# fani-lab/OpeNTF

Hardware: AMD Instinct MI355X
Metric: teams/sec (train) bnn_emb d=128 on DBLP (higher is better)
Workload: dtype f32 (fp16x3 split products, f32 accumulate)

## Files before the change

opentf_amd/csrc/ntf_device.h:

```cpp
#pragma once
#include <hip/hip_runtime.h>
#include <stdint.h>
#include "ntf_kernels.h"

namespace ntf {

typedef float f32x16 __attribute__((ext_vector_type(16)));
typedef float f32x4 __attribute__((ext_vector_type(4)));

__device__ __forceinline__ uint32_t fmix32(uint32_t x) {
    x ^= x >> 16; x *= 0x85ebca6bu; x ^= x >> 13; x *= 0xc2b2ae35u; x ^= x >> 16;
    return x;
}

__device__ __forceinline__ uint32_t sign_word(uint32_t k0, uint32_t k1, uint32_t r, uint32_t cb) {
    uint32_t h = fmix32(r * 0x9E3779B1u + k0);
    return fmix32(h ^ (cb * 0x85EBCA77u + k1));
}
__device__ __forceinline__ float sign_hash(uint32_t k0, uint32_t k1, uint32_t r, uint32_t c) {
    return ((sign_word(k0, k1, r, c >> 5) >> (c & 31)) & 1u) ? -1.0f : 1.0f;
}
__device__ __forceinline__ float sign_at(const SignSpec& s, int64_t r, int64_t c) {
    if (s.inj) return s.inj[r * s.ld + c];
    return sign_hash(s.k0, s.k1, (uint32_t)r, (uint32_t)c);
// ... 115 lines not shown
    const float denom = fmaf(__builtin_amdgcn_sqrtf(v), inv_bc2_sqrt, eps);
    p = p - (lr_over_bc1 * m) * __builtin_amdgcn_rcpf(denom);
#endif
}

__device__ __forceinline__ float wave_reduce_sum(float v) {
#pragma unroll
    for (int o = 32; o > 0; o >>= 1) v += __shfl_xor(v, o, 64);
    return v;
}
__device__ __forceinline__ double wave_reduce_sum_d(double v) {
#pragma unroll
    for (int o = 32; o > 0; o >>= 1) v += __shfl_xor(v, o, 64);
    return v;
}
__device__ __forceinline__ float block_reduce_sum(float v) {
    __shared__ float sh_f[16];
    v = wave_reduce_sum(v);
    const int w = threadIdx.x >> 6, nw = (blockDim.x + 63) >> 6;
    __syncthreads();
    if ((threadIdx.x & 63) == 0) sh_f[w] = v;
    __syncthreads();
    float s = 0.f;
    if (threadIdx.x == 0) for (int i = 0; i < nw; ++i) s += sh_f[i];
    return s;
}
__device__ __forceinline__ double block_reduce_sum_d(double v) {
    __shared__ double sh_d[16];
    v = wave_reduce_sum_d(v);
    const int w = threadIdx.x >> 6, nw = (blockDim.x + 63) >> 6;
// ... 10 lines not shown
```

opentf_amd/csrc/ntf_engine.hip:

```cpp
#include "../../include/opentf_amd.h"
#include "ntf_kernels.h"
#include "ntf_fused.h"
#include "ntf_head.h"
#include "ntf_host.h"
#include "ntf_select.h"

#include <algorithm>
#include <cmath>
#include <cstdio>
#include <cstdlib>
#include <cstring>
#include <string>
#include <vector>

using namespace ntf;

static thread_local std::string g_create_error;

struct LayerInfo {
    int in = 0, out = 0;
    int64_t off[4] = {0, 0, 0, 0};
    int64_t nw() const { return (int64_t)in * out; }
};

// ... 91 lines not shown
    int64_t pre_used = 0;
    int eval_chain = 0; bool chain_valid = false; double* d_chain = nullptr;
    bool join_pending = false;
    bool pre_rotated = false;
    bool fin_pend = false; NormalSpec fin_eps; float fin_klw = 0.f;
    int (*cb_fn)(int32_t, void*) = nullptr; void* cb_user = nullptr;
    bool pend_valid = false; FusedDw pend; NormalSpec pend_eps_b; float pend_klw_b = 0.f; int pend_chunks = 0;
    std::vector<int32_t> ub_entries; void* ub_host[2] = {nullptr, nullptr}; char* ub_dev[2] = {nullptr, nullptr}; hipEvent_t ub_ev[2] = {nullptr, nullptr};
    bool ub_used[2] = {false, false}; size_t ub_cap = 0; int ub_slot = 0; int ub_nsup[2] = {0, 0}; double ub_total[2] = {0, 0};
    uint16_t* pl_mu = nullptr; uint16_t* pl_wp = nullptr;
    hipStream_t st2 = nullptr;
    hipEvent_t ev_chunk = nullptr, ev_side = nullptr;
    hipStream_t st3 = nullptr; hipEvent_t ev_fork = nullptr, ev_join = nullptr;
    hipStream_t st4 = nullptr; hipEvent_t ev_aux = nullptr;
    int side_bwd = 1;
    bool ep = false; int ep_lo = 0, Mg = 0, ep_world = 1;
    bool ep_side = false;
    int ep_open = 0; StepCtx ep_ctx;
};

static int join_side(ntf_engine* e);

struct Scope {
    ntf_engine* e; int fam; hipEvent_t a = nullptr, b = nullptr;
    bool on() const {
        const bool fwd = fam == F_OUT_FUSED_FWD || fam == F_OUT_FWD, dw = fam == F_OUT_FUSED_DW || fam == F_OUT_BWD_DW;
        return e->timing == 1 || (e->timing == 2 && (fwd || dw)) || (e->timing == 3 && fwd) || (e->timing == 4 && dw);
    }
    Scope(ntf_engine* e_, int f) : e(e_), fam(f) {
        if (!on()) return;
// ... 67 lines not shown
    if (const char* hp = getenv("NTF_HEAD_PREFETCH")) e->head_prefetch = atoi(hp);
    if (const char* pf = getenv("NTF_PREFETCH")) e->prefetch = atoi(pf);
    if (const char* hd = getenv("NTF_HEAD")) e->head = atoi(hd);
    if (const char* mb = getenv("NTF_MERGE_BIAS")) e->merge_bias = atoi(mb);
    if (const char* sw = getenv("NTF_L0_SWEEP")) e->l0_sweep = atoi(sw);
    if (const char* fp = getenv("NTF_FNN_PIPE")) e->fnn_pipe = atoi(fp);
    if (const char* mh = getenv("NTF_MH_HEAD")) e->mh_head = atoi(mh);
    if (const char* ek = getenv("NTF_EVAL_KERNEL")) e->eval_kernel = atoi(ek);
    if (const char* nf = getenv("NTF_INFER_F32")) e->infer_f32 = atoi(nf);
    if (const char* mc = getenv("NTF_INFER_MC")) e->infer_mc = atoi(mc);
    if (const char* mb = getenv("NTF_INFER_MC_BYTES")) e->infer_mc_bytes = atoll(mb);
    if (const char* fc = getenv("NTF_F32_COPY_MERGED")) e->f32_copy_merged = atoi(fc);
    if (const char* eh = getenv("NTF_EP_HEAD_PREFETCH")) e->ep_head_prefetch = atoi(eh);
    if (const char* dr = getenv("NTF_DP_RANGES")) e->dp_ranges = atoi(dr);
    if (const char* ds = getenv("NTF_DP_SIDE_BWD")) e->dp_side_bwd = atoi(ds);
    if (const char* sb = getenv("NTF_SIDE_BWD")) e->side_bwd = atoi(sb);
    if (cfg->stream) e->st = (hipStream_t)cfg->stream;
    else { if (hipStreamCreate(&e->st) != hipSuccess) { g_create_error = "hipStreamCreate failed"; delete e; return NTF_EHIP; } e->own_stream = true; }
    int64_t off = 0;
    auto seg = [&](int64_t n) { int64_t o = off; off += (n + 63) / 64 * 64; return o; };
    e->layers.resize(e->L);
    for (int l = 0; l < e->L; ++l) {
        LayerInfo& li = e->layers[l];
        li.in = cfg->dims[l]; li.out = cfg->dims[l + 1];
        li.off[NTF_P_WEIGHT] = seg(li.nw());
        li.off[NTF_P_BIAS] = seg(li.out);
        if (cfg->bayesian) { li.off[NTF_P_RHO_WEIGHT] = seg(li.nw()); li.off[NTF_P_RHO_BIAS] = seg(li.out); }
        if (l < e->L - 1) e->maxhid = std::max(e->maxhid, li.out);
    }
    e->n_params = off;
// ... 17 lines not shown
    const int B = cfg->max_batch, M = cfg->dims[e->L];
    int rc = NTF_OK;
    auto A = [&](int r) { if (rc == NTF_OK) rc = r; };
    A(dev_alloc(e, &e->P, off)); A(dev_alloc(e, &e->G, off)); A(dev_alloc(e, &e->M1, off)); A(dev_alloc(e, &e->V2, off));
    A(dev_alloc(e, &e->d_rows, B)); for (int k = 0; k < 2; ++k) A(dev_alloc(e, &e->d_neg_set[k], (int64_t)B * std::max(1, cfg->ns)));
    e->act.assign(e->L, nullptr);
    for (int l = (cfg->input_mode == NTF_INPUT_MULTIHOT ? 1 : 0); l < e->L; ++l) A(dev_alloc(e, &e->act[l], (int64_t)B * cfg->dims[l]));
    A(dev_alloc(e, &e->Zout, (int64_t)B * M)); A(dev_alloc(e, &e->dZout, (int64_t)((M + 255) / 256 * 256) * fused_ldb(B)));
    if (e->maxhid) { A(dev_alloc(e, &e->Zh, (int64_t)B * e->maxhid)); A(dev_alloc(e, &e->dAct[0], (int64_t)B * e->maxhid)); A(dev_alloc(e, &e->dAct[1], (int64_t)B * e->maxhid)); }
    e->Wp.assign(e->L, nullptr); e->bp.assign(e->L, nullptr);
    if (cfg->bayesian) for (int l = 0; l < e->L; ++l) { A(dev_alloc(e, &e->Wp[l], e->layers[l].nw())); A(dev_alloc(e, &e->bp[l], e->layers[l].out)); }
    A(dev_alloc(e, &e->partial, (int64_t)B * std::max(loss_dense_nchunk(M), fused_loss_slots(M)))); A(dev_alloc(e, &e->row_fix, B));
    if (cfg->bayesian && cfg->input_mode == NTF_INPUT_MULTIHOT) A(dev_alloc(e, &e->l0_touched, (int64_t)(cfg->dims[0] + 255) / 256 * 256));
    A(dev_alloc(e, &e->d_loss, 4)); A(dev_alloc(e, &e->d_kl, 4)); A(dev_alloc(e, &e->d_chain, 2)); A(dev_alloc(e, &e->d_acc, 2)); A(dev_alloc(e, &e->d_acc_steps, 2));
    A(dev_alloc(e, &e->ent_mc, B)); A(dev_alloc(e, &e->ent_mean, B)); A(dev_alloc(e, &e->gemm_slab, kGemmSlabFloats));
    if (rc == NTF_OK && fused_ok(e)) {
        A(dev_alloc(e, &e->dh_slab, fused_dh_slab_floats(B, e->layers[e->L - 1].in, M)));
        for (int k = 0; k < 2; ++k) A(dev_alloc(e, &e->fws_set[k], (int64_t)fused_workspace_bytes(B, e->layers[e->L - 1].in, M)));
        e->fws = e->fws_set[0];
        if (cfg->mfma != NTF_MFMA_F32 && e->layers[e->L - 1].in == 128) {
            A(dev_alloc(e, &e->pl_mu, fused_planes_elems(M, 128)));
            if (cfg->bayesian) A(dev_alloc(e, &e->pl_wp, fused_planes_elems(M, 128)));
            if (rc == NTF_OK) { hipMemsetAsync(e->pl_mu, 0, (size_t)fused_planes_elems(M, 128) * 2, e->st); if (e->pl_wp) hipMemsetAsync(e->pl_wp, 0, (size_t)fused_planes_elems(M, 128) * 2, e->st); }
        }
    }
    e->inj_eps_w.assign(e->L, nullptr); e->inj_eps_b.assign(e->L, nullptr); e->inj_s_in.assign(e->L, nullptr); e->inj_s_out.assign(e->L, nullptr);
    if (rc != NTF_OK) { g_create_error = e->err; ntf_engine_destroy(e); return rc; }
    hipMemsetAsync(e->P, 0, off * 4, e->st); hipMemsetAsync(e->G, 0, off * 4, e->st);
    hipMemsetAsync(e->M1, 0, off * 4, e->st); hipMemsetAsync(e->V2, 0, off * 4, e->st);
    hipMemsetAsync(e->d_acc, 0, 16, e->st); hipMemsetAsync(e->d_acc_steps, 0, 16, e->st);
    hipMemsetAsync(e->d_kl, 0, 32, e->st);
    e->d_range = reinterpret_cast<int32_t*>(e->d_kl + 1);
    if (hipStreamSynchronize(e->st) != hipSuccess) { g_create_error = "device initialisation failed"; ntf_engine_destroy(e); return NTF_EHIP; }
    *out = e;
    return NTF_OK;
}

extern "C" void ntf_engine_destroy(ntf_engine* e) {
    if (!e) return;
    hipSetDevice(e->cfg.device);
    if (e->st) hipStreamSynchronize(e->st);
    if (e->st4) { hipStreamSynchronize(e->st4); hipStreamDestroy(e->st4); hipEventDestroy(e->ev_aux); }
    if (e->st3) { hipStreamSynchronize(e->st3); hipStreamDestroy(e->st3); hipEventDestroy(e->ev_fork); hipEventDestroy(e->ev_join); }
    if (e->st2) { hipStreamSynchronize(e->st2); hipStreamDestroy(e->st2); hipEventDestroy(e->ev_chunk); hipEventDestroy(e->ev_side); }
    dfree(e->P); dfree(e->G); dfree(e->M1); dfree(e->V2);
    dfree(e->m_indptr); dfree(e->m_indices); dfree(e->s_indptr); dfree(e->s_indices); dfree(e->table); dfree(e->Xall);
    dfree(e->al_prob); dfree(e->al_alias); dfree(e->al_weight);
    dfree(e->d_rows); dfree(e->d_order); dfree(e->d_neg_set[0]); dfree(e->d_neg_set[1]);
    for (auto& p : e->act) dfree(p);
    dfree(e->Zout); dfree(e->dZout); dfree(e->Pbuf); dfree(e->Zh); dfree(e->dAct[0]); dfree(e->dAct[1]);
    for (auto& p : e->Wp) dfree(p);
    for (auto& p : e->bp) dfree(p);
    dfree(e->l0_touched);
    dfree(e->mc_ring); dfree(e->mc_bp); dfree(e->mc_hz); dfree(e->mc_lossp);
    dfree(e->partial); dfree(e->row_fix); dfree(e->d_loss); dfree(e->d_kl); dfree(e->d_chain); dfree(e->d_acc); dfree(e->d_acc_steps);
    dfree(e->ent_mc); dfree(e->ent_mean); dfree(e->dh_slab); dfree(e->fws_set[0]); dfree(e->fws_set[1]); dfree(e->pl_mu); dfree(e->pl_wp); dfree(e->gemm_slab); dfree(e->tk_vals); dfree(e->tk_idx);
    for (auto* v : {&e->inj_eps_w, &e->inj_eps_b, &e->inj_s_in, &e->inj_s_out}) for (auto& p : *v) dfree(p);
    for (auto& r : e->recs) { hipEventDestroy(r.a); hipEventDestroy(r.b); }
    for (auto ev : e->pool) hipEventDestroy(ev);
    for (int k = 0; k < 2; ++k) { if (e->ub_host[k]) hipHostFree(e->ub_host[k]); if (e->ub_dev[k]) hipFree(e->ub_dev[k]); if (e->ub_ev[k]) hipEventDestroy(e->ub_ev[k]); }
    if (e->own_stream && e->st) hipStreamDestroy(e->st);
    delete e;
}

static int upload_csr(ntf_engine* e, const int64_t* indptr, const int32_t* indices, int64_t n_rows, int64_t** d_ip, int32_t** d_ix, int width) {
    if (!indptr || n_rows < 0) FAIL(e, NTF_EINVAL, "csr: bad arguments");
    const int64_t nnz = indptr[n_rows];
    if (nnz < 0 || (nnz > 0 && !indices)) FAIL(e, NTF_EINVAL, "csr: bad arguments");
    for (int64_t i = 0; i < n_rows; ++i) if (indptr[i + 1] < indptr[i]) FAIL(e, NTF_EINVAL, "csr: indptr not monotone");
    for (int64_t p = 0; p < nnz; ++p) if (indices[p] < 0 || indices[p] >= width) FAIL(e, NTF_EINVAL, "csr: column id out of range");
    HIPCHK(e, hipSetDevice(e->cfg.device));
// ... 506 lines not shown
        const SignSpec so = sign_spec(e, n, e->L - 1, T_S_OUT, lo.out);
        Scope t(e, F_OUT_FUSED_AUX); launch_fused_prep_planes(e->st, n.B, lo.in, M, 1, ws_next, kH16Scale, &so, 0, 1);
    }
    HIPCHK(e, hipEventRecord(e->ev_aux, e->st4));
    e->st = head_st;
    { Scope t(e, F_GEMM_HIDDEN); head_launch(e, e->st, n, ws_next, true, e->d_kl + 2, false, range_ptr(e) ? e->d_range + 4 : nullptr, true, e->pre0_step == n.step); }
    e->hp.valid = true; e->hp.step = n.step; e->hp.rows = n.rows_dev; e->hp.B = n.B; e->hp.ub = ub_next;
    return NTF_OK;
}
static bool head_prefetch_possible(const ntf_engine* e, const StepCtx& c, int B) {
    const bool can_head = (mh_head_ok(e) && !e->ep) || (e->head && e->L == 2 && e->cfg.input_mode != NTF_INPUT_MULTIHOT && head_supported(e->cfg.dims[0], e->cfg.dims[1]) &&
                          (e->cfg.mfma == NTF_MFMA_DEFAULT || e->cfg.mfma == NTF_MFMA_FP16X3));
    if (!e->cfg.bayesian && !e->fnn_pipe) return false;
    return e->head_prefetch && can_head && c.fuse_adam && e->cfg.fuse_adam == 1 && e->pre_valid && e->pre_step == c.step + 1 && e->hp_next_B > 0 && !c.inj &&
           (e->cfg.nsd != NTF_NSD_UNIGRAM_B || e->hp_next_host != nullptr) && c.global_B == B;
}

static int run_step(ntf_engine* e, const StepCtx& c, bool accumulate_epoch) {
    int r;
    const int B = c.B, M = e->cfg.dims[e->L];
    const float inv_B = 1.0f / (float)c.global_B;
    const LayerInfo& lo = e->layers[e->L - 1];
    const bool fused = fused_ok(e);
    const double out_nw = (double)e->Mg * lo.in, out_nb = (double)e->Mg;
    int nslots;
    const int64_t* neg = (e->cfg.nsd != NTF_NSD_NONE && e->cfg.ns > 0) ? e->d_neg_set[c.step & 1] : nullptr;
    bool prod_side = false, aux = false, swt_aux = false, loss_side = false, use_pre = false;
    const bool use_head = fused && c.part <= 1 && !c.inj &&
                          ((mh_head_ok(e) && !e->ep) || (e->head && e->L == 2 && e->cfg.input_mode != NTF_INPUT_MULTIHOT && head_supported(e->cfg.dims[0], e->cfg.dims[1]) &&
                                                         (e->cfg.mfma == NTF_MFMA_DEFAULT || e->cfg.mfma == NTF_MFMA_FP16X3)));
// ... 175 lines not shown
        }
    }
    bool l0_sweep_now = false;
    for (int l = e->L - 1; l >= 0; --l) {
        const LayerInfo& li = e->layers[l];
        const bool last = (l == e->L - 1);
        if (c.part == 2 && !last) break;
        if (c.part == 3 && last) continue;
        if (side && l == e->L - 2) e->st = e->st3;
        const float* in = e->act[l];
        float* gW = e->G + li.off[NTF_P_WEIGHT]; float* gb = e->G + li.off[NTF_P_BIAS];
        float* gRW = e->cfg.bayesian ? e->G + li.off[NTF_P_RHO_WEIGHT] : nullptr;
        float* gRb = e->cfg.bayesian ? e->G + li.off[NTF_P_RHO_BIAS] : nullptr;
        SignSpec sin_, sout_;
        if (e->cfg.bayesian) { sin_ = sign_spec(e, c, l, T_S_IN, li.in); sout_ = sign_spec(e, c, l, T_S_OUT, li.out); }
        if (last && fused) {
            FusedDw f;
            f.B = B; f.H = li.in; f.M = M; f.bayes = e->cfg.bayesian;
            f.dzT = e->dZout; f.h = in; f.g_mu = gW; f.g_rho = gRW; f.g_b = gb; f.g_bp = gRb; f.ws = e->fws;
            f.mu = e->P + li.off[NTF_P_WEIGHT];
            f.s_out = sout_; f.s_out_inj = e->cfg.bayesian && (sout_.inj != nullptr || sin_.inj != nullptr);
            f.split = e->cfg.mfma != NTF_MFMA_F32 && split_products(e);
            f.a_scale = dz_scale16(e, c.global_B); f.h_scale = kH16Scale; f.rflag = range_ptr(e);
            f.dz_packed = f.split && li.in == 128 && e->pl_mu != nullptr;
            e->last_dz_packed_scale = f.dz_packed ? f.a_scale : 0.f;
            if (f.dz_packed && !c.defer_dw && !(c.fuse_adam && e->cfg.fuse_adam == 2)) {
                const int tiles = (M + fused_dw_tile() - 1) / fused_dw_tile(), nib = fused_ldb(B) / 32;
                int ks = e->dw_ksplit > 0 ? e->dw_ksplit : (tiles <= 128 ? std::min({256 / tiles, 8, std::max(1, nib / 4)}) : 1);
                while (ks > 1 && fused_dw_part_floats(M, li.in, ks) > (int64_t)e->cfg.max_batch * M) --ks;
                if (ks > 1) { f.ksplit = ks; f.part = e->Zout; }
// ... 40 lines not shown
                    StepCtx nx; nx.step = c.step + 1;
                    f.produce = 1; f.lean = e->lean; f.nx_eps = normal_spec(e, nx, l, T_EPS_W); f.nx_wp = e->Wp[l]; f.nx_pl_wp = e->pl_wp; f.nx_pl_mu = e->pl_mu; f.nx_pscale = kW16Scale;
                    f.nx_klw = 1.0 / out_nw; f.nx_kl = e->d_kl + 2; f.nx_rflag = e->d_range + 4;
                    e->pre_valid = true; e->pre_step = c.step + 1;
                }
                if (e->prefetch && e->fnn_pipe && !e->cfg.bayesian && f.dz_packed && e->pl_mu && range_ptr(e)) {
                    f.produce = 1; f.nx_pl_mu = e->pl_mu; f.nx_pl_wp = nullptr; f.nx_pscale = kW16Scale; f.nx_kl = e->d_kl + 2; f.nx_rflag = e->d_range + 4;
                    e->pre_valid = true; e->pre_step = c.step + 1;
                }
                if (e->cfg.bayesian) { e->fin_pend = true; e->fin_eps = normal_spec(e, c, l, T_EPS_B); e->fin_klw = kl_share / ((float)out_nb * (float)c.global_B); }
            }
            { Scope t(e, F_OUT_FUSED_DW); launch_fused_out_dw(e->st, f); }
        dw_done:;
        } else {
            const float* dZ = last ? e->dZout : e->dAct[(l + 1) & 1];
            { Scope t(e, F_BIAS_GRAD); launch_bias_grad(e->st, dZ, li.out, B, li.out, sout_, gb, gRb, e->gemm_slab, kGemmSlabFloats); }
            if (l == 0 && e->cfg.input_mode == NTF_INPUT_MULTIHOT) {
                Scope t(e, F_MULTIHOT);
                l0_sweep_now = e->l0_sweep && e->cfg.bayesian && c.fuse_adam && e->adam_in_dw && !c.defer_dw && c.part == 0 && !e->ep && e->l0_touched &&
                               (li.nw() & 3) == 0 && (li.out & 3) == 0;
                if (!(l0_sweep_now && e->g0_clean)) {
                    HIPCHK(e, hipMemsetAsync(gW, 0, (size_t)li.nw() * 4, e->st));
                    if (gRW) HIPCHK(e, hipMemsetAsync(gRW, 0, (size_t)li.nw() * 4, e->st));
                }
                e->g0_clean = false; e->pre0_step = ~0ull;
                if (l0_sweep_now) HIPCHK(e, hipMemsetAsync(e->l0_touched, 0, (size_t)li.in, e->st));
                launch_multihot_bwd(e->st, c.rows_dev, B, li.in, li.out, e->s_indptr, e->s_indices, dZ, sin_, sout_, gW, gRW, l0_sweep_now ? e->l0_touched : nullptr);
            } else {
                Scope t(e, last ? F_OUT_BWD_DW : F_GEMM_HIDDEN);
                GemmArgs g;
                g.M = li.out; g.N = li.in; g.K = B;
                g.A = dZ; g.sam = 1; g.sak = li.out;
                g.B = in; g.sbk = li.in; g.sbn = 1;
                g.C = gW; g.ldc = li.in;
                const int wtiles = ((li.out + 63) / 64) * ((li.in + 63) / 64);
                if (wtiles < 64 && B >= 256) { g.ksplit = std::max(1, std::min({B >= 2048 ? 64 : 16, B / 64, (int)(kGemmSlabFloats / ((int64_t)li.out * li.in))})); g.slab = e->gemm_slab; }
                if (g.ksplit <= 1) { g.ksplit = 1; g.slab = nullptr; }
                launch_gemm(e->st, g);
                if (e->cfg.bayesian) { g.sa = sout_; g.sa_t = 1; g.sb = sin_; g.sb_t = 0; g.C = gRW; launch_gemm(e->st, g); }
            }
            if (l > 0) {
                Scope t(e, last ? F_OUT_BWD_DA : F_GEMM_HIDDEN);
                float* dA = e->dAct[l & 1];
                GemmArgs g;
                g.M = B; g.N = li.in; g.K = li.out;
                g.A = dZ; g.sam = li.out; g.sak = 1;
                g.B = e->P + li.off[NTF_P_WEIGHT]; g.sbk = li.in; g.sbn = 1;
                g.C = dA; g.ldc = li.in;
                g.mask = e->act[l]; g.ldmask = li.in;
                const int tiles = ((B + 63) / 64) * ((li.in + 63) / 64);
                int ks = 1;
                if (li.out >= 4096) ks = std::max(1, std::min({64, 1024 / tiles, (int)(kGemmSlabFloats / ((int64_t)B * li.in))}));
                g.ksplit = ks; g.slab = e->gemm_slab;
                launch_gemm(e->st, g);
// ... 9 lines not shown
            if (l == 0 && l0_sweep_now) {
                FlipoutSweep a;
                a.mu = e->P + li.off[NTF_P_WEIGHT]; a.rho = e->P + li.off[NTF_P_RHO_WEIGHT]; a.g_mu = gW; a.g_rho = gRW;
                a.m_mu = e->M1 + li.off[NTF_P_WEIGHT]; a.v_mu = e->V2 + li.off[NTF_P_WEIGHT]; a.m_rho = e->M1 + li.off[NTF_P_RHO_WEIGHT]; a.v_rho = e->V2 + li.off[NTF_P_RHO_WEIGHT];
                a.n = li.nw(); a.eps = normal_spec(e, c, l, T_EPS_W); a.klw = kl_share / ((float)li.nw() * (float)c.global_B);
                const double b1 = 0.9, b2 = 0.999, tt = (double)(e->adam_t + 1);
                a.lr = e->lr; a.b1 = (float)b1; a.b2 = (float)b2; a.adam_eps = 1e-8f; a.bc1 = (float)(1.0 - std::pow(b1, tt)); a.bc2_sqrt = (float)std::sqrt(1.0 - std::pow(b2, tt));
                StepCtx nx; nx.step = c.step + 1;
                const bool produce = e->pre_valid && e->pre_step == c.step + 1;
                a.nx_eps = normal_spec(e, nx, l, T_EPS_W); a.nx_wp = e->Wp[l]; a.nx_klw = 1.0 / (double)li.nw(); a.nx_kl = produce ? e->d_kl + 2 : nullptr;
                a.touched = e->l0_touched; a.H = li.out;
                launch_flipout_sweep(e->st, a);
                e->l0_swept = true; e->g0_clean = true;
                if (produce) e->pre0_step = c.step + 1;
            } else
            if (!(last && fused))
                launch_flipout_grad_finalize(e->st, e->P + li.off[NTF_P_WEIGHT], e->P + li.off[NTF_P_RHO_WEIGHT], gW, gRW, li.nw(),
                                             normal_spec(e, c, l, T_EPS_W), kl_share / ((float)li.nw() * (float)c.global_B));
            if (!(last && e->fin_pend))
            launch_flipout_grad_finalize(e->st, e->P + li.off[NTF_P_BIAS], e->P + li.off[NTF_P_RHO_BIAS], gb, gRb, li.out,
                                         normal_spec(e, c, l, T_EPS_B), kl_share / ((last ? (float)out_nb : (float)li.out) * (float)c.global_B));
        }
    }
    if (side) {
        if (head_prefetch_possible(e, c, B) && !e->ep) {
            if ((r = prefetch_next_head(e, c, e->st3, e->ev_fork))) return r;
            e->st = e->st3;
        }
        if (e->hp.valid && e->hp.step == c.step + 1) HIPCHK(e, hipStreamWaitEvent(e->st3, e->ev_aux, 0));
        HIPCHK(e, hipEventRecord(e->ev_join, e->st3));
        e->st = restore.main;
        if (c.defer_dw) e->join_pending = true;
        else HIPCHK(e, hipStreamWaitEvent(e->st, e->ev_join, 0));
    }
// ... 835 lines not shown
```

opentf_amd/csrc/ntf_kernels.h:

```cpp
#pragma once
#include <hip/hip_runtime.h>
#include <stddef.h>
#include <stdint.h>

namespace ntf {

constexpr float kLeakySlope = 0.01f;

struct SignSpec {
    const float* inj = nullptr;
    int64_t ld = 0;
    uint32_t k0 = 0, k1 = 0;
    int enabled = 0;
};

struct NormalSpec {
    const float* inj = nullptr;
    uint32_t k0 = 0, k1 = 0, tag = 0, step = 0;
    int64_t qbase = 0;
};

struct GemmArgs {
    int M = 0, N = 0, K = 0;
    const float* A = nullptr; int64_t sam = 0, sak = 0;
    const float* B = nullptr; int64_t sbk = 0, sbn = 0;
    SignSpec sa; int sa_t = 0;
    SignSpec sb; int sb_t = 0;
    float* C = nullptr; int64_t ldc = 0;
    float* Act = nullptr; int64_t ldact = 0;
    const float* bias = nullptr;
    SignSpec sc;
    const float* mask = nullptr; int64_t ldmask = 0;
    int accumulate = 0;
    int ksplit = 1;
    float* slab = nullptr;
    float alpha = 1.0f;
};

void launch_gemm(hipStream_t st, const GemmArgs& a);

void launch_gather_meanpool(hipStream_t st, const int64_t* indptr, const int32_t* indices, const float* table,
                            const int64_t* rows, int64_t n, int d, int mean, float* out);
void launch_gather_dense_rows(hipStream_t st, const float* X, int d, const int64_t* rows, int64_t n, float* out);
void launch_multihot_fwd(hipStream_t st, const int64_t* rows, int B, int S, int H, const int64_t* indptr, const int32_t* indices,
                         const float* W, const float* b, const float* Wp , const float* bp, SignSpec sin, SignSpec sout, float* act);
void launch_multihot_bwd(hipStream_t st, const int64_t* rows, int B, int S, int H, const int64_t* indptr, const int32_t* indices,
                         const float* dZ, SignSpec sin, SignSpec sout, float* gW , float* gWp , uint8_t* touched = nullptr);

struct PerturbChain { double* kl_out2 = nullptr; int* mu_flag_out = nullptr; const int* raise_if = nullptr; };
void launch_flipout_perturb(hipStream_t st, const float* rho, const float* mu, int64_t n, NormalSpec eps, float* out, double w, double* kl_out,
                            uint16_t* planes_w = nullptr, uint16_t* planes_mu = nullptr, const float* pmu = nullptr, int H = 0,
                            float pscale = 1.f,
                            int* rflag = nullptr ,
                            const int* only_if = nullptr ,
// ... 66 lines not shown
```

opentf_amd/csrc/ntf_kernels.hip:

```cpp
#include "ntf_kernels.h"
#include <cstdlib>
#include "ntf_device.h"
#include "ntf_select.h"
#include <algorithm>
#include <cstdint>

namespace ntf {

constexpr int GBM = 64, GBN = 64, GBK = 32, GLD = GBK + 1;

__global__ __launch_bounds__(256) void k_gemm(GemmArgs a) {
    __shared__ float As[GBM * GLD];
    __shared__ float Bs[GBN * GLD];
    const int tid = threadIdx.x, lane = tid & 63, wave = tid >> 6;
    const int m0 = blockIdx.y * GBM, n0 = blockIdx.x * GBN;
    int kper = (a.K + a.ksplit - 1) / a.ksplit;
    kper = (kper + GBK - 1) / GBK * GBK;
    const int kbeg = blockIdx.z * kper;
    const int kend = min(a.K, kbeg + kper);
    const bool a_kc = (a.sak == 1), b_nc = (a.sbn == 1);
    f32x16 acc;
#pragma unroll
    for (int i = 0; i < 16; ++i) acc[i] = 0.f;
    const int wm = wave >> 1, wn = wave & 1;
// ... 253 lines not shown
    const int blocks = (int)std::min<int64_t>((quads + 255) / 256, only_if ? 256 : 2048);
    hipLaunchKernelGGL(k_flipout_perturb, dim3(blocks), dim3(256), 0, st, rho, mu, n, eps, out, w, kl_out, planes_w, planes_mu, pmu, H, pscale, planes_w ? rflag : nullptr, only_if, ch);
}

__global__ void k_flipout_grad_finalize(const float* __restrict__ mu, const float* __restrict__ rho, float* __restrict__ g_mu,
                                        float* __restrict__ g_rho, int64_t n, NormalSpec eps, float klw) {
    const int64_t q = (int64_t)blockIdx.x * blockDim.x + threadIdx.x;
    const int64_t e0 = q * 4;
    if (e0 >= n) return;
    float z[4];
    normal4(eps, q, e0, n, z);
#pragma unroll
    for (int j = 0; j < 4; ++j) {
        const int64_t e = e0 + j;
        if (e >= n) break;
        const RhoTerms t = rho_terms(rho[e]);
        g_rho[e] = g_rho[e] * z[j] * t.sg + klw * t.kl_a * t.kl_b;
        g_mu[e] += klw * mu[e];
    }
}
void launch_flipout_grad_finalize(hipStream_t st, const float* mu, const float* rho, float* g_mu, float* g_rho, int64_t n,
                                  NormalSpec eps, float klw) {
    if (n <= 0) return;
    const int64_t quads = (n + 3) / 4;
    hipLaunchKernelGGL(k_flipout_grad_finalize, dim3((unsigned)((quads + 255) / 256)), dim3(256), 0, st, mu, rho, g_mu, g_rho, n, eps, klw);
}

__global__ void k_kl_value(const float* __restrict__ mu, const float* __restrict__ rho, int64_t n, double w, double* out) {
    double s = 0.0;
    for (int64_t e = (int64_t)blockIdx.x * blockDim.x + threadIdx.x; e < n; e += (int64_t)gridDim.x * blockDim.x) {
        const float sigma = softplus_rho(rho[e]);
        const float m = mu[e];
        s += (double)(-logf(sigma) + 0.5f * (sigma * sigma + m * m) - 0.5f);
// ... 93 lines not shown
    const int n = blockIdx.x * 256 + threadIdx.x;
    if (n >= N) return;
    float s1 = 0.f, s2 = 0.f;
    for (int b = 0; b < B; ++b) {
        const float v = dZ[(int64_t)b * ld + n];
        s1 += v;
        if (g_pert) s2 += v * sign_at(sout, b, n);
    }
    g_b[n] = s1;
    if (g_pert) g_pert[n] = s2;
}
__global__ __launch_bounds__(256) void k_bias_grad_wave(const float* __restrict__ dZ, int64_t ld, int B, int N, SignSpec sout,
                                                        float* __restrict__ g_b, float* __restrict__ g_pert) {
    const int n = blockIdx.x * 4 + (threadIdx.x >> 6), lane = threadIdx.x & 63;
    if (n >= N) return;
    float s1 = 0.f, s2 = 0.f;
    for (int b = lane; b < B; b += 64) {
        const float v = dZ[(int64_t)b * ld + n];
        s1 += v;
        if (g_pert) s2 += v * sign_at(sout, b, n);
    }
    s1 = wave_reduce_sum(s1); s2 = wave_reduce_sum(s2);
    if (lane == 0) { g_b[n] = s1; if (g_pert) g_pert[n] = s2; }
}
__global__ __launch_bounds__(256) void k_bias_grad_rows(const float* __restrict__ dZ, int64_t ld, int B, int N, SignSpec sout, float* __restrict__ part, int has_pert) {
    const int b0 = blockIdx.x * 32, b1 = min(B, b0 + 32);
    for (int n = threadIdx.x; n < N; n += 256) {
        float s1 = 0.f, s2 = 0.f;
#pragma unroll 8
        for (int b = b0; b < b1; ++b) {
            const float v = dZ[(int64_t)b * ld + n];
            s1 += v;
            if (has_pert) s2 += v * sign_at(sout, b, n);
        }
        part[((int64_t)blockIdx.x * 2) * N + n] = s1;
        if (has_pert) part[((int64_t)blockIdx.x * 2 + 1) * N + n] = s2;
    }
// ... 496 lines not shown
```

Measured before the change: 697,200.

## Fuse hidden-layer weight/bias grad, split-K reduce and flipout finalize into one kernel

Adds a single hidden-layer backward kernel that computes the mean and sign-perturbed weight gradients with f32 MFMA split-K, reduces the slices in the last-arriving block via atomic tickets, and applies the flipout/KL finalize inline. Extra blocks in the same grid compute the bias gradient and bias finalize. This replaces separate bias-grad, two GEMM, split-K reduce and two finalize launches for small hidden layers, cutting launch overhead and round trips through global memory. The cost is a ticket counter protocol with threadfences, a fixed ticket array of 16 entries, and an eligibility gate that sends larger layers down the old path.

New measurement: 689,200. -1.1%, worse.

```diff
diff --git a/opentf_amd/csrc/ntf_device.h b/opentf_amd/csrc/ntf_device.h
--- a/opentf_amd/csrc/ntf_device.h
+++ b/opentf_amd/csrc/ntf_device.h
@@ -153,6 +153,23 @@
     for (int o = 32; o > 0; o >>= 1) v += __shfl_xor(v, o, 64);
     return v;
 }
+__device__ __forceinline__ void flipout_grad_finalize_one(float& g_mu, float& g_rho, float mu, float rho, float z, float klw) {
+#pragma clang fp contract(off)
+    const RhoTerms t = rho_terms(rho);
+    const float chain = g_rho * z * t.sg, kl = klw * t.kl_a * t.kl_b;
+    g_rho = chain + kl;
+    g_mu = fmaf(klw, mu, g_mu);
+}
+__device__ __forceinline__ void bias_grad_column(const float* __restrict__ dZ, int64_t ld, int B, int n, int lane, const SignSpec& sout, bool pert, float& s1, float& s2) {
+    s1 = 0.f; s2 = 0.f;
+    for (int b = lane; b < B; b += 64) {
+        const float v = dZ[(int64_t)b * ld + n];
+        s1 += v;
+        if (pert) s2 += v * sign_at(sout, b, n);
+    }
+    s1 = wave_reduce_sum(s1); s2 = wave_reduce_sum(s2);
+}
+
 __device__ __forceinline__ float block_reduce_sum(float v) {
     __shared__ float sh_f[16];
     v = wave_reduce_sum(v);
diff --git a/opentf_amd/csrc/ntf_engine.hip b/opentf_amd/csrc/ntf_engine.hip
--- a/opentf_amd/csrc/ntf_engine.hip
+++ b/opentf_amd/csrc/ntf_engine.hip
@@ -129,6 +129,8 @@
     hipStream_t st3 = nullptr; hipEvent_t ev_fork = nullptr, ev_join = nullptr;
     hipStream_t st4 = nullptr; hipEvent_t ev_aux = nullptr;
     int side_bwd = 1;
+    int hidden_bwd = 1;
+    uint32_t* hb_tickets = nullptr;
     bool ep = false; int ep_lo = 0, Mg = 0, ep_world = 1;
     bool ep_side = false;
     int ep_open = 0; StepCtx ep_ctx;
@@ -226,6 +228,7 @@
     if (const char* eh = getenv("NTF_EP_HEAD_PREFETCH")) e->ep_head_prefetch = atoi(eh);
     if (const char* dr = getenv("NTF_DP_RANGES")) e->dp_ranges = atoi(dr);
     if (const char* ds = getenv("NTF_DP_SIDE_BWD")) e->dp_side_bwd = atoi(ds);
+    if (const char* hb = getenv("NTF_HIDDEN_BWD")) e->hidden_bwd = atoi(hb);
     if (const char* sb = getenv("NTF_SIDE_BWD")) e->side_bwd = atoi(sb);
     if (cfg->stream) e->st = (hipStream_t)cfg->stream;
     else { if (hipStreamCreate(&e->st) != hipSuccess) { g_create_error = "hipStreamCreate failed"; delete e; return NTF_EHIP; } e->own_stream = true; }
@@ -273,6 +276,7 @@
     if (cfg->bayesian && cfg->input_mode == NTF_INPUT_MULTIHOT) A(dev_alloc(e, &e->l0_touched, (int64_t)(cfg->dims[0] + 255) / 256 * 256));
     A(dev_alloc(e, &e->d_loss, 4)); A(dev_alloc(e, &e->d_kl, 4)); A(dev_alloc(e, &e->d_chain, 2)); A(dev_alloc(e, &e->d_acc, 2)); A(dev_alloc(e, &e->d_acc_steps, 2));
     A(dev_alloc(e, &e->ent_mc, B)); A(dev_alloc(e, &e->ent_mean, B)); A(dev_alloc(e, &e->gemm_slab, kGemmSlabFloats));
+    A(dev_alloc(e, &e->hb_tickets, hidden_bwd_tickets()));
     if (rc == NTF_OK && fused_ok(e)) {
         A(dev_alloc(e, &e->dh_slab, fused_dh_slab_floats(B, e->layers[e->L - 1].in, M)));
         for (int k = 0; k < 2; ++k) A(dev_alloc(e, &e->fws_set[k], (int64_t)fused_workspace_bytes(B, e->layers[e->L - 1].in, M)));
@@ -288,7 +292,7 @@
     hipMemsetAsync(e->P, 0, off * 4, e->st); hipMemsetAsync(e->G, 0, off * 4, e->st);
     hipMemsetAsync(e->M1, 0, off * 4, e->st); hipMemsetAsync(e->V2, 0, off * 4, e->st);
     hipMemsetAsync(e->d_acc, 0, 16, e->st); hipMemsetAsync(e->d_acc_steps, 0, 16, e->st);
-    hipMemsetAsync(e->d_kl, 0, 32, e->st);
+    hipMemsetAsync(e->d_kl, 0, 32, e->st); hipMemsetAsync(e->hb_tickets, 0, (size_t)hidden_bwd_tickets() * 4, e->st);
     e->d_range = reinterpret_cast<int32_t*>(e->d_kl + 1);
     if (hipStreamSynchronize(e->st) != hipSuccess) { g_create_error = "device initialisation failed"; ntf_engine_destroy(e); return NTF_EHIP; }
     *out = e;
@@ -313,7 +317,7 @@
     dfree(e->l0_touched);
     dfree(e->mc_ring); dfree(e->mc_bp); dfree(e->mc_hz); dfree(e->mc_lossp);
     dfree(e->partial); dfree(e->row_fix); dfree(e->d_loss); dfree(e->d_kl); dfree(e->d_chain); dfree(e->d_acc); dfree(e->d_acc_steps);
-    dfree(e->ent_mc); dfree(e->ent_mean); dfree(e->dh_slab); dfree(e->fws_set[0]); dfree(e->fws_set[1]); dfree(e->pl_mu); dfree(e->pl_wp); dfree(e->gemm_slab); dfree(e->tk_vals); dfree(e->tk_idx);
+    dfree(e->ent_mc); dfree(e->ent_mean); dfree(e->dh_slab); dfree(e->fws_set[0]); dfree(e->fws_set[1]); dfree(e->pl_mu); dfree(e->pl_wp); dfree(e->gemm_slab); dfree(e->hb_tickets); dfree(e->tk_vals); dfree(e->tk_idx);
     for (auto* v : {&e->inj_eps_w, &e->inj_eps_b, &e->inj_s_in, &e->inj_s_out}) for (auto& p : *v) dfree(p);
     for (auto& r : e->recs) { hipEventDestroy(r.a); hipEventDestroy(r.b); }
     for (auto ev : e->pool) hipEventDestroy(ev);
@@ -850,6 +854,12 @@
     if (!e->cfg.bayesian && !e->fnn_pipe) return false;
     return e->head_prefetch && can_head && c.fuse_adam && e->cfg.fuse_adam == 1 && e->pre_valid && e->pre_step == c.step + 1 && e->hp_next_B > 0 && !c.inj &&
            (e->cfg.nsd != NTF_NSD_UNIGRAM_B || e->hp_next_host != nullptr) && c.global_B == B;
+}
+
+static int hidden_gemm_ksplit(const LayerInfo& li, int B) {
+    const int wtiles = ((li.out + 63) / 64) * ((li.in + 63) / 64);
+    if (!(wtiles < 64 && B >= 256)) return 1;
+    return std::max(1, std::min({B >= 2048 ? 64 : 16, B / 64, (int)(kGemmSlabFloats / ((int64_t)li.out * li.in))}));
 }
 
 static int run_step(ntf_engine* e, const StepCtx& c, bool accumulate_epoch) {
@@ -1055,6 +1065,7 @@
         float* gRb = e->cfg.bayesian ? e->G + li.off[NTF_P_RHO_BIAS] : nullptr;
         SignSpec sin_, sout_;
         if (e->cfg.bayesian) { sin_ = sign_spec(e, c, l, T_S_IN, li.in); sout_ = sign_spec(e, c, l, T_S_OUT, li.out); }
+        bool hb_done = false;
         if (last && fused) {
             FusedDw f;
             f.B = B; f.H = li.in; f.M = M; f.bayes = e->cfg.bayesian;
@@ -1125,6 +1136,24 @@
         dw_done:;
         } else {
             const float* dZ = last ? e->dZout : e->dAct[(l + 1) & 1];
+            const int hb_ks = hidden_gemm_ksplit(li, B);
+            hb_done = e->hidden_bwd && !last && c.part == 0 && !e->ep && c.global_B == B && !(l == 0 && e->cfg.input_mode == NTF_INPUT_MULTIHOT) &&
+                      hb_ks > 1 && B < 1024 && li.in % 32 == 0 && li.out % 32 == 0 && li.in <= 256 && li.out <= 256 &&
+                      (int64_t)2 * gemm_live_slices(B, hb_ks) * li.nw() <= kGemmSlabFloats;
+            if (hb_done) {
+                Scope t(e, F_GEMM_HIDDEN);
+                HiddenBwd h;
+                h.dZ = dZ; h.X = in; h.B = B; h.out = li.out; h.in = li.in; h.ksplit = hb_ks; h.bayes = e->cfg.bayesian;
+                h.sout = sout_; h.sin = sin_; h.gW = gW; h.gRW = gRW; h.gb = gb; h.gRb = gRb;
+                h.mu_w = e->P + li.off[NTF_P_WEIGHT]; h.mu_b = e->P + li.off[NTF_P_BIAS];
+                if (e->cfg.bayesian) {
+                    h.rho_w = e->P + li.off[NTF_P_RHO_WEIGHT]; h.rho_b = e->P + li.off[NTF_P_RHO_BIAS];
+                    h.eps_w = normal_spec(e, c, l, T_EPS_W); h.klw_w = kl_share / ((float)li.nw() * (float)c.global_B);
+                    h.eps_b = normal_spec(e, c, l, T_EPS_B); h.klw_b = kl_share / ((float)li.out * (float)c.global_B);
+                }
+                h.slab = e->gemm_slab; h.tickets = e->hb_tickets;
+                launch_hidden_bwd(e->st, h);
+            } else {
             { Scope t(e, F_BIAS_GRAD); launch_bias_grad(e->st, dZ, li.out, B, li.out, sout_, gb, gRb, e->gemm_slab, kGemmSlabFloats); }
             if (l == 0 && e->cfg.input_mode == NTF_INPUT_MULTIHOT) {
                 Scope t(e, F_MULTIHOT);
@@ -1144,11 +1173,11 @@
                 g.A = dZ; g.sam = 1; g.sak = li.out;
                 g.B = in; g.sbk = li.in; g.sbn = 1;
                 g.C = gW; g.ldc = li.in;
-                const int wtiles = ((li.out + 63) / 64) * ((li.in + 63) / 64);
-                if (wtiles < 64 && B >= 256) { g.ksplit = std::max(1, std::min({B >= 2048 ? 64 : 16, B / 64, (int)(kGemmSlabFloats / ((int64_t)li.out * li.in))})); g.slab = e->gemm_slab; }
-                if (g.ksplit <= 1) { g.ksplit = 1; g.slab = nullptr; }
+                g.ksplit = hidden_gemm_ksplit(li, B);
+                g.slab = g.ksplit > 1 ? e->gemm_slab : nullptr;
                 launch_gemm(e->st, g);
                 if (e->cfg.bayesian) { g.sa = sout_; g.sa_t = 1; g.sb = sin_; g.sb_t = 0; g.C = gRW; launch_gemm(e->st, g); }
+            }
             }
             if (l > 0) {
                 Scope t(e, last ? F_OUT_BWD_DA : F_GEMM_HIDDEN);
@@ -1188,10 +1217,10 @@
                 e->l0_swept = true; e->g0_clean = true;
                 if (produce) e->pre0_step = c.step + 1;
             } else
-            if (!(last && fused))
+            if (!(last && fused) && !hb_done)
                 launch_flipout_grad_finalize(e->st, e->P + li.off[NTF_P_WEIGHT], e->P + li.off[NTF_P_RHO_WEIGHT], gW, gRW, li.nw(),
                                              normal_spec(e, c, l, T_EPS_W), kl_share / ((float)li.nw() * (float)c.global_B));
-            if (!(last && e->fin_pend))
+            if (!(last && e->fin_pend) && !hb_done)
             launch_flipout_grad_finalize(e->st, e->P + li.off[NTF_P_BIAS], e->P + li.off[NTF_P_RHO_BIAS], gb, gRb, li.out,
                                          normal_spec(e, c, l, T_EPS_B), kl_share / ((last ? (float)out_nb : (float)li.out) * (float)c.global_B));
         }
diff --git a/opentf_amd/csrc/ntf_hidden_bwd.hip b/opentf_amd/csrc/ntf_hidden_bwd.hip
--- /dev/null
+++ b/opentf_amd/csrc/ntf_hidden_bwd.hip
@@ -0,0 +1,149 @@
+#include "ntf_kernels.h"
+#include "ntf_device.h"
+
+namespace ntf {
+
+constexpr int HT = 64, HK = 32;
+
+__device__ __forceinline__ float hb_flip(float v, uint32_t bit) { return __uint_as_float(__float_as_uint(v) ^ (bit << 31)); }
+__device__ __forceinline__ float4 hb_signed(float4 v, const SignSpec& s, int row, int col) {
+    if (s.inj) {
+        const float* g = s.inj + (int64_t)row * s.ld + col;
+        return make_float4(v.x * g[0], v.y * g[1], v.z * g[2], v.w * g[3]);
+    }
+    const uint32_t w = sign_word(s.k0, s.k1, (uint32_t)row, (uint32_t)col >> 5) >> (col & 31);
+    return make_float4(hb_flip(v.x, w & 1u), hb_flip(v.y, (w >> 1) & 1u), hb_flip(v.z, (w >> 2) & 1u), hb_flip(v.w, (w >> 3) & 1u));
+}
+
+template <bool BAYES>
+__device__ __forceinline__ void hb_load_row(const HiddenBwd& a, int gk, int kend, bool a_in, bool b_in, int ca, int cb, float4& ra, float4& rb, float4& ras, float4& rbs) {
+    ra = rb = ras = rbs = make_float4(0.f, 0.f, 0.f, 0.f);
+    if (gk >= kend) return;
+    if (a_in) { ra = *reinterpret_cast<const float4*>(a.dZ + (int64_t)gk * a.out + ca); if (BAYES) ras = hb_signed(ra, a.sout, gk, ca); }
+    if (b_in) { rb = *reinterpret_cast<const float4*>(a.X + (int64_t)gk * a.in + cb); if (BAYES) rbs = hb_signed(rb, a.sin, gk, cb); }
+}
+
+template <bool BAYES>
+__global__ __launch_bounds__(256) void k_hidden_bwd(HiddenBwd a, int kper, int nslice, int tiles_n, int ntile) {
+    __shared__ float sA[HK * HT], sB[HK * HT];
+    __shared__ float sAs[BAYES ? HK * HT : 4], sBs[BAYES ? HK * HT : 4];
+    __shared__ float s_bias[8];
+    __shared__ int s_last;
+    const int tid = threadIdx.x, lane = tid & 63, wave = tid >> 6;
+    const int nprod = ntile * nslice;
+
+    if ((int)blockIdx.x >= nprod) {
+        const int q = (int)blockIdx.x - nprod, n = q * 4 + wave;
+        float s1, s2;
+        bias_grad_column(a.dZ, a.out, a.B, n, lane, a.sout, BAYES, s1, s2);
+        if (!BAYES) { if (lane == 0) a.gb[n] = s1; return; }
+        if (lane == 0) { s_bias[wave] = s1; s_bias[4 + wave] = s2; }
+        __syncthreads();
+        if (tid == 0) {
+            float z[4];
+            normal4(a.eps_b, q, (int64_t)q * 4, a.out, z);
+#pragma unroll
+            for (int j = 0; j < 4; ++j) {
+                float gm = s_bias[j], gr = s_bias[4 + j];
+                flipout_grad_finalize_one(gm, gr, a.mu_b[q * 4 + j], a.rho_b[q * 4 + j], z[j], a.klw_b);
+                a.gb[q * 4 + j] = gm; a.gRb[q * 4 + j] = gr;
+            }
+        }
+        return;
+    }
+
+    const int tile = (int)blockIdx.x % ntile, z = (int)blockIdx.x / ntile;
+    const int m0 = (tile / tiles_n) * HT, n0 = (tile % tiles_n) * HT;
+    const int kbeg = z * kper, kend = min(a.B, kbeg + kper);
+    const int nstep = (kend - kbeg + HK - 1) / HK;
+    const int wm = wave >> 1, wn = wave & 1;
+    const bool live = m0 + wm * 32 < a.out && n0 + wn * 32 < a.in;
+    const int sr = tid >> 4, sc = (tid & 15) * 4;
+    const bool a_in = m0 + sc < a.out, b_in = n0 + sc < a.in;
+
+    float4 ra0, ra1, rb0, rb1, ras0, ras1, rbs0, rbs1;
+#define HB_LOAD(s) do { \
+        hb_load_row<BAYES>(a, kbeg + (s) * HK + sr, kend, a_in, b_in, m0 + sc, n0 + sc, ra0, rb0, ras0, rbs0); \
+        hb_load_row<BAYES>(a, kbeg + (s) * HK + sr + 16, kend, a_in, b_in, m0 + sc, n0 + sc, ra1, rb1, ras1, rbs1); } while (0)
+
+    f32x16 acc, accs;
+#pragma unroll
+    for (int i = 0; i < 16; ++i) { acc[i] = 0.f; accs[i] = 0.f; }
+    HB_LOAD(0);
+    for (int s = 0; s < nstep; ++s) {
+        if (s) __syncthreads();
+        const int o0 = sr * HT + sc, o1 = (sr + 16) * HT + sc;
+        *reinterpret_cast<float4*>(&sA[o0]) = ra0; *reinterpret_cast<float4*>(&sB[o0]) = rb0;
+        *reinterpret_cast<float4*>(&sA[o1]) = ra1; *reinterpret_cast<float4*>(&sB[o1]) = rb1;
+        if (BAYES) {
+            *reinterpret_cast<float4*>(&sAs[o0]) = ras0; *reinterpret_cast<float4*>(&sBs[o0]) = rbs0;
+            *reinterpret_cast<float4*>(&sAs[o1]) = ras1; *reinterpret_cast<float4*>(&sBs[o1]) = rbs1;
+        }
+        __syncthreads();
+        if (s + 1 < nstep) HB_LOAD(s + 1);
+        if (live) {
+            const int fa = (lane >> 5) * HT + wm * 32 + (lane & 31), fb = (lane >> 5) * HT + wn * 32 + (lane & 31);
+#pragma unroll
+            for (int kk = 0; kk < HK / 2; ++kk) {
+                acc = __builtin_amdgcn_mfma_f32_32x32x2f32(sA[fa + 2 * kk * HT], sB[fb + 2 * kk * HT], acc, 0, 0, 0);
+                if (BAYES) accs = __builtin_amdgcn_mfma_f32_32x32x2f32(sAs[fa + 2 * kk * HT], sBs[fb + 2 * kk * HT], accs, 0, 0, 0);
+            }
+        }
+    }
+
+#undef HB_LOAD
+
+    const int64_t mn = (int64_t)a.out * a.in;
+    float* const slab_w = a.slab;
+    float* const slab_r = a.slab + (int64_t)nslice * mn;
+    if (live) {
+        const int col = n0 + wn * 32 + (lane & 31);
+#pragma unroll
+        for (int r = 0; r < 16; ++r) {
+            const int row = m0 + wm * 32 + (r & 3) + 8 * (r >> 2) + 4 * (lane >> 5);
+            slab_w[(int64_t)z * mn + (int64_t)row * a.in + col] = acc[r];
+            if (BAYES) slab_r[(int64_t)z * mn + (int64_t)row * a.in + col] = accs[r];
+        }
+    }
+    __threadfence();
+    __syncthreads();
+    if (tid == 0) s_last = atomicAdd(&a.tickets[tile], 1u) == (uint32_t)(nslice - 1);
+    __syncthreads();
+    if (!s_last) return;
+    __threadfence();
+#pragma unroll
+    for (int i = 0; i < HT * HT / 4 / 256; ++i) {
+        const int qid = tid + 256 * i, row = m0 + (qid >> 4), col = n0 + (qid & 15) * 4;
+        if (row >= a.out || col >= a.in) continue;
+        const int64_t e0 = (int64_t)row * a.in + col;
+        float4 gw = make_float4(0.f, 0.f, 0.f, 0.f), gr = gw;
+        for (int s = 0; s < nslice; ++s) {
+            const float4 p = *reinterpret_cast<const float4*>(slab_w + (int64_t)s * mn + e0);
+            gw.x += p.x; gw.y += p.y; gw.z += p.z; gw.w += p.w;
+            if (BAYES) {
+                const float4 t = *reinterpret_cast<const float4*>(slab_r + (int64_t)s * mn + e0);
+                gr.x += t.x; gr.y += t.y; gr.z += t.z; gr.w += t.w;
+            }
+        }
+        if (BAYES) {
+            float zn[4];
+            normal4(a.eps_w, e0 >> 2, e0, mn, zn);
+            const float4 mu = *reinterpret_cast<const float4*>(a.mu_w + e0), rho = *reinterpret_cast<const float4*>(a.rho_w + e0);
+            flipout_grad_finalize_one(gw.x, gr.x, mu.x, rho.x, zn[0], a.klw_w); flipout_grad_finalize_one(gw.y, gr.y, mu.y, rho.y, zn[1], a.klw_w);
+            flipout_grad_finalize_one(gw.z, gr.z, mu.z, rho.z, zn[2], a.klw_w); flipout_grad_finalize_one(gw.w, gr.w, mu.w, rho.w, zn[3], a.klw_w);
+            *reinterpret_cast<float4*>(a.gRW + e0) = gr;
+        }
+        *reinterpret_cast<float4*>(a.gW + e0) = gw;
+    }
+    if (tid == 0) atomicExch(&a.tickets[tile], 0u);
+}
+
+void launch_hidden_bwd(hipStream_t st, const HiddenBwd& a) {
+    const int kper = gemm_slice_rows(a.B, a.ksplit), nslice = gemm_live_slices(a.B, a.ksplit);
+    const int tiles_n = (a.in + HT - 1) / HT, ntile = ((a.out + HT - 1) / HT) * tiles_n;
+    const dim3 grid((unsigned)(ntile * nslice + a.out / 4));
+    if (a.bayes) hipLaunchKernelGGL(k_hidden_bwd<true>, grid, dim3(256), 0, st, a, kper, nslice, tiles_n, ntile);
+    else hipLaunchKernelGGL(k_hidden_bwd<false>, grid, dim3(256), 0, st, a, kper, nslice, tiles_n, ntile);
+}
+
+}
diff --git a/opentf_amd/csrc/ntf_kernels.h b/opentf_amd/csrc/ntf_kernels.h
--- a/opentf_amd/csrc/ntf_kernels.h
+++ b/opentf_amd/csrc/ntf_kernels.h
@@ -38,6 +38,20 @@
 };
 
 void launch_gemm(hipStream_t st, const GemmArgs& a);
+inline int gemm_slice_rows(int K, int ksplit) { return ((K + ksplit - 1) / ksplit + 31) / 32 * 32; }
+inline int gemm_live_slices(int K, int ksplit) { const int kper = gemm_slice_rows(K, ksplit); return (K + kper - 1) / kper; }
+
+struct HiddenBwd {
+    const float* dZ = nullptr; const float* X = nullptr;
+    int B = 0, out = 0, in = 0, ksplit = 1, bayes = 0;
+    SignSpec sout, sin;
+    float *gW = nullptr, *gRW = nullptr, *gb = nullptr, *gRb = nullptr;
+    const float *mu_w = nullptr, *rho_w = nullptr, *mu_b = nullptr, *rho_b = nullptr;
+    NormalSpec eps_w, eps_b; float klw_w = 0.f, klw_b = 0.f;
+    float* slab = nullptr; uint32_t* tickets = nullptr;
+};
+constexpr int hidden_bwd_tickets() { return 16; }
+void launch_hidden_bwd(hipStream_t st, const HiddenBwd& a);
 
 void launch_gather_meanpool(hipStream_t st, const int64_t* indptr, const int32_t* indices, const float* table,
                             const int64_t* rows, int64_t n, int d, int mean, float* out);
diff --git a/opentf_amd/csrc/ntf_kernels.hip b/opentf_amd/csrc/ntf_kernels.hip
--- a/opentf_amd/csrc/ntf_kernels.hip
+++ b/opentf_amd/csrc/ntf_kernels.hip
@@ -291,9 +291,9 @@
     for (int j = 0; j < 4; ++j) {
         const int64_t e = e0 + j;
         if (e >= n) break;
-        const RhoTerms t = rho_terms(rho[e]);
-        g_rho[e] = g_rho[e] * z[j] * t.sg + klw * t.kl_a * t.kl_b;
-        g_mu[e] += klw * mu[e];
+        float gm = g_mu[e], gr = g_rho[e];
+        flipout_grad_finalize_one(gm, gr, mu[e], rho[e], z[j], klw);
+        g_rho[e] = gr; g_mu[e] = gm;
     }
 }
 void launch_flipout_grad_finalize(hipStream_t st, const float* mu, const float* rho, float* g_mu, float* g_rho, int64_t n,
@@ -417,13 +417,8 @@
                                                         float* __restrict__ g_b, float* __restrict__ g_pert) {
     const int n = blockIdx.x * 4 + (threadIdx.x >> 6), lane = threadIdx.x & 63;
     if (n >= N) return;
-    float s1 = 0.f, s2 = 0.f;
-    for (int b = lane; b < B; b += 64) {
-        const float v = dZ[(int64_t)b * ld + n];
-        s1 += v;
-        if (g_pert) s2 += v * sign_at(sout, b, n);
-    }
-    s1 = wave_reduce_sum(s1); s2 = wave_reduce_sum(s2);
+    float s1, s2;
+    bias_grad_column(dZ, ld, B, n, lane, sout, g_pert != nullptr, s1, s2);
     if (lane == 0) { g_b[n] = s1; if (g_pert) g_pert[n] = s2; }
 }
 __global__ __launch_bounds__(256) void k_bias_grad_rows(const float* __restrict__ dZ, int64_t ld, int B, int N, SignSpec sout, float* __restrict__ part, int has_pert) {
```
